# tugitbartlomiej/ViTParticleFilterTracker

Hardware: AMD Instinct MI355X
Metric: frames/sec @ 4096 particles, ViT-B/16 224px; 1/2/4/8 MI355X scaling (higher is better)
Workload: dtype bf16; 1 GPU; 4096 particles, vit_base_patch16_224 bf16, 224x224 frames, full tracking step per frame; particles=4096, particles_per_gpu=4096, arch=vit_base_patch16_224, hip_graph=True, parallelism=particle-shard x1

## Files before the change

vitparticlefiltertracker_amd/csrc/gemm_bf16.hip:

```cpp
#include <algorithm>
#include <atomic>
#include "gemm_common.h"

using namespace vpf;
using namespace vpf::gemm;

namespace {

constexpr int BK = 64;
constexpr int OPERAND_BYTES = BM * BK * 2;
static_assert(OPERAND_BYTES == TILE_BYTES, "bf16 K-tile geometry");
constexpr int AUX_PARTS = 15;
constexpr int MAX_PARTS = 16;
constexpr int AUX_BYTES = 2048 + AUX_PARTS * 2048;

template <int EPI, bool WIDE = false, bool OUT8 = false, bool PART = false>
__global__ __launch_bounds__(NTHREADS) void k_gemm_bf16(const bf16_t* __restrict__ A, int lda,
                                                        const bf16_t* __restrict__ W,
                                                        const float* __restrict__ bias,
                                                        const bf16_t* residual,
                                                        const float* __restrict__ pos, int g2,
                                                        const float2* __restrict__ stats,
                                                        const float* __restrict__ colsum,
                                                        bf16_t* C, int ldc, int M, int N, int K, int group,
// ... 131 lines not shown
    const int region = (wid >> 1) + ((wid >> 1) >= (nk % 3) ? 1 : 0);
    finish_tile<EPI, OUT8, DIRECT>(smem + region * OPERAND_BYTES + (wid & 1) * 16384, aux, acc, wm, wn, m0, n0, lane,
                                   residual, pos, g2, C, ldc, M, N, stats_out, stats_rows, o8);
}

template <int EPI, bool OUT8 = false>
__global__ __launch_bounds__(NTHREADS) void k_gemm_pp(const bf16_t* __restrict__ A, int lda,
                                                      const bf16_t* __restrict__ W,
                                                      const float* __restrict__ bias,
                                                      const bf16_t* residual,
                                                      const float* __restrict__ pos, int g2,
                                                      const float2* __restrict__ stats,
                                                      const float* __restrict__ colsum,
                                                      bf16_t* C, int ldc, int M, int N, int K, int group,
                                                      int stats_parts, float ln_eps, float* stats_out,
                                                      int stats_rows, Out8 o8) {
    constexpr int HALF = 16384;
    constexpr int RING = 8 * HALF;
    static_assert(RING + AUX_BYTES <= 160 * 1024, "LDS budget");
    __shared__ __attribute__((aligned(16))) char smem[RING + AUX_BYTES];
    const int tid = threadIdx.x, lane = tid & 63;
    const int wid = __builtin_amdgcn_readfirstlane(tid >> 6);
    const int wm = wid >> 2, wn = wid & 3;

    int m0, n0;
    tile_of(M, N, group, m0, n0);
    constexpr bool DIRECT = (EPI == VPF_EPI_LN_GELU || EPI == VPF_EPI_BIAS_GELU) && !OUT8;

    const char* Ablk = reinterpret_cast<const char*>(A) + (size_t)m0 * lda * 2;
    const char* Bblk = reinterpret_cast<const char*>(W) + (size_t)n0 * K * 2;
    uint32_t off[4][2];
#pragma unroll
    for (int p = 0; p < 2; ++p) {
        const int rho = (wid + 8 * p) * 8 + (lane >> 3);
        const int lch = (lane & 7) ^ ((rho >> 1) & 7);
        const int ra0 = (rho >> 6) * 128 + (rho & 63);
        const int rb0 = (rho >> 5) * 64 + (DIRECT ? wperm(rho & 31) : (rho & 31));
        const int ra[2] = {ra0, ra0 + 64}, rb[2] = {rb0, rb0 + 32};
#pragma unroll
        for (int h = 0; h < 2; ++h) {
            off[h == 0 ? 0 : 3][p] = (uint32_t)min(ra[h], M - 1 - m0) * (uint32_t)(lda * 2) + (uint32_t)(lch * 16);
            off[h == 0 ? 1 : 2][p] = (uint32_t)min(rb[h], N - 1 - n0) * (uint32_t)(K * 2) + (uint32_t)(lch * 16);
        }
    }
    const int nk = K / BK;
    auto stage = [&](int type, int kt) {
        kt = min(kt, nk - 1);
        char* slot = smem + ((kt & 1) * 4 + type) * HALF;
        const char* src = (type == 0 || type == 3) ? Ablk : Bblk;
        const uint32_t koff = (uint32_t)kt * (BK * 2);
#pragma unroll
        for (int p = 0; p < 2; ++p)
            __builtin_amdgcn_global_load_lds((gptr_t)(src + off[type][p] + koff), (lptr_t)(slot + (wid + 8 * p) * 1024),
                                             16, 0, 0);
    };

    constexpr bool LN = (EPI == VPF_EPI_LN || EPI == VPF_EPI_LN_GELU);
    char* aux = smem + RING;
    dma_bias_colsum<LN>(aux, bias, colsum, n0, N, wid, lane);
    if constexpr (LN) dma_planes(aux + 2048, stats, stats_parts, m0, M, wid, lane);
    stage(0, 0); stage(1, 0); stage(2, 0); stage(3, 0); stage(0, 1); stage(1, 1);
    asm volatile("s_waitcnt vmcnt(8)" ::: "memory");
    __builtin_amdgcn_s_barrier();
    if (wm == 1) __builtin_amdgcn_s_barrier();
    asm volatile("" ::: "memory");

    f32x4 acc[4][8];
#pragma unroll
    for (int j = 0; j < 4; ++j)
#pragma unroll
        for (int i = 0; i < 8; ++i) acc[j][i] = f32x4{0.f, 0.f, 0.f, 0.f};

    const int fr = lane & 15, fq = lane >> 4;
    const int sw = (fr >> 1) & 7;
    const int abase = (wm * 64 + fr) * 128, bbase = (wn * 32 + fr) * 128;
    auto mfma_quadrant = [&](const i32x4 (&fa)[2][4], const i32x4 (&fb)[2][2], int mh, int nh) {
        asm volatile("s_waitcnt lgkmcnt(0)" ::: "memory");
        __builtin_amdgcn_sched_barrier(0);
#pragma unroll
        for (int ks = 0; ks < 2; ++ks)
#pragma unroll
            for (int j = 0; j < 2; ++j)
#pragma unroll
                for (int i = 0; i < 4; ++i)
                    acc[nh * 2 + j][mh * 4 + i] = __builtin_amdgcn_mfma_f32_16x16x32_bf16(
                        __builtin_bit_cast(bf16x8, fb[ks][j]), __builtin_bit_cast(bf16x8, fa[ks][i]),
                        acc[nh * 2 + j][mh * 4 + i], 0, 0, 0);
        __builtin_amdgcn_sched_barrier(0);
    };
    auto read_a = [&](i32x4 (&fa)[2][4], const char* slot) {
#pragma unroll
        for (int ks = 0; ks < 2; ++ks)
#pragma unroll
            for (int i = 0; i < 4; ++i) fa[ks][i] = lds16(slot + abase + i * 2048 + (((ks * 4 + fq) ^ sw) << 4));
    };
    auto read_b = [&](i32x4 (&fb)[2][2], const char* slot) {
#pragma unroll
        for (int ks = 0; ks < 2; ++ks)
#pragma unroll
            for (int j = 0; j < 2; ++j) fb[ks][j] = lds16(slot + bbase + j * 2048 + (((ks * 4 + fq) ^ sw) << 4));
    };
    auto bar = [&]() {
        __builtin_amdgcn_sched_barrier(0);
        __builtin_amdgcn_s_barrier();
        __builtin_amdgcn_sched_barrier(0);
    };

    for (int kt = 0; kt < nk; ++kt) {
        const char* buf = smem + (kt & 1) * 4 * HALF;
        i32x4 fa0[2][4], fa1[2][4], fb0[2][2], fb1[2][2];
        read_a(fa0, buf);
        read_b(fb0, buf + HALF);
        stage(2, kt + 1);
        asm volatile("s_waitcnt vmcnt(8)" ::: "memory");
        bar();
        mfma_quadrant(fa0, fb0, 0, 0);
        bar();
        read_b(fb1, buf + 2 * HALF);
        stage(3, kt + 1);
        asm volatile("s_waitcnt vmcnt(8)" ::: "memory");
        bar();
        mfma_quadrant(fa0, fb1, 0, 1);
        bar();
        read_a(fa1, buf + 3 * HALF);
        stage(0, kt + 2);
        bar();
        mfma_quadrant(fa1, fb1, 1, 1);
        bar();
        stage(1, kt + 2);
        asm volatile("s_waitcnt vmcnt(8)" ::: "memory");
        bar();
        mfma_quadrant(fa1, fb0, 1, 0);
        bar();
    }
    if (wm == 0) __builtin_amdgcn_s_barrier();
    asm volatile("s_waitcnt vmcnt(0)" ::: "memory");

    if constexpr (LN) combine_planes(aux + 2048, aux, stats_parts, K, ln_eps, tid);
    finish_tile<EPI, OUT8, DIRECT>(smem + wid * 16384, aux, acc, wm, wn, m0, n0, lane, residual, pos, g2, C, ldc, M, N,
                                   stats_out, stats_rows, o8);
}

constexpr int WALK_HALF = 16384;
constexpr int WALK_RING = 8 * WALK_HALF;
constexpr int WALK_GROUP_IMG = 2048;
constexpr int walk_aux_set(int epi) { return epi == VPF_EPI_BIAS_RESIDUAL ? 1024 : 4096; }
constexpr int walk_smem(int epi) {
    return WALK_RING + 2 * walk_aux_set(epi) + (epi_is_gelu(epi) ? 0 : 8 * WALK_GROUP_IMG);
}
constexpr bool walk_reads_early(int epi) {
    return epi == VPF_EPI_LN || epi == VPF_EPI_LN_GELU || epi == VPF_EPI_BIAS_RESIDUAL;
}

template <int OFF>
__device__ __forceinline__ i32x4 lds16_at(uint32_t addr) {
    static_assert(OFF >= 0 && OFF < 65536, "ds_read offset field");
    i32x4 v;
    asm volatile("ds_read_b128 %0, %1 offset:%2" : "=v"(v) : "v"(addr), "n"(OFF));
    return v;
}
template <int SLOT, int NF>
__device__ __forceinline__ void frag_read(i32x4 (&f)[2][NF], const uint32_t (&ad)[2]) {
#pragma unroll
    for (int ks = 0; ks < 2; ++ks) {
        f[ks][0] = lds16_at<SLOT>(ad[ks]);
        f[ks][1] = lds16_at<SLOT + 2048>(ad[ks]);
        if constexpr (NF == 4) {
            f[ks][2] = lds16_at<SLOT + 4096>(ad[ks]);
            f[ks][3] = lds16_at<SLOT + 6144>(ad[ks]);
        }
    }
}

template <int EPI, bool EARLY = walk_reads_early(EPI)>
__device__ __forceinline__ void gemm_walk_body(char* smem, const bf16_t* __restrict__ A, int lda,
                                               const bf16_t* __restrict__ W, const float* __restrict__ bias,
                                               const float2* __restrict__ stats, const float* __restrict__ colsum,
                                               const bf16_t* residual, bf16_t* C, int ldc, int M, int N, int K,
                                               int group, int tiles, float* stats_out) {
    constexpr bool RES = EPI == VPF_EPI_BIAS_RESIDUAL;
    constexpr bool DIRECT = epi_is_gelu(EPI);
    constexpr int HALF = WALK_HALF;
    constexpr int RING = WALK_RING;
    constexpr int AUX_SET = walk_aux_set(EPI);
    constexpr int GROUP_IMG = WALK_GROUP_IMG;
    const int tid = threadIdx.x, lane = tid & 63;
    const int wid = __builtin_amdgcn_readfirstlane(tid >> 6);
    const int wm = wid >> 2, wn = wid & 3;
    constexpr bool LN = epi_is_ln(EPI);
    const int nk = K / BK;

    const int stride = (int)gridDim.x >> 3;
    int lid = xcd_first(tiles, (int)blockIdx.x & 7) + ((int)blockIdx.x >> 3);
    const int lid_end = xcd_first(tiles, ((int)blockIdx.x & 7) + 1);
    if (lid >= lid_end) return;
    int m0, n0;
    tile_of_lid(M, N, group, lid, m0, n0);

    const char* Ablk;
    const char* Bblk;
    uint32_t off[4][2];
    auto set_panels = [&](int tm0, int tn0, int ln) {
        Ablk = reinterpret_cast<const char*>(A) + (size_t)tm0 * lda * 2;
        Bblk = reinterpret_cast<const char*>(W) + (size_t)tn0 * K * 2;
#pragma unroll
        for (int p = 0; p < 2; ++p) {
            const int rho = (wid + 8 * p) * 8 + (ln >> 3);
            const int lch = (ln & 7) ^ ((rho >> 1) & 7);
            const int ra0 = (rho >> 6) * 128 + (rho & 63);
            const int rb0 = (rho >> 5) * 64 + (DIRECT ? wperm(rho & 31) : (rho & 31));
            const int ra[2] = {ra0, ra0 + 64}, rb[2] = {rb0, rb0 + 32};
#pragma unroll
            for (int h = 0; h < 2; ++h) {
                off[h == 0 ? 0 : 3][p] = (uint32_t)min(ra[h], M - 1 - tm0) * (uint32_t)(lda * 2) + (uint32_t)(lch * 16);
                off[h == 0 ? 1 : 2][p] = (uint32_t)min(rb[h], N - 1 - tn0) * (uint32_t)(K * 2) + (uint32_t)(lch * 16);
            }
        }
    };
    auto stage = [&](int type, int kt) {
        kt = min(kt, nk - 1);
        char* slot = smem + ((kt & 1) * 4 + type) * HALF;
        const char* src = (type == 0 || type == 3) ? Ablk : Bblk;
        const uint32_t koff = (uint32_t)kt * (BK * 2);
#pragma unroll
        for (int p = 0; p < 2; ++p)
            __builtin_amdgcn_global_load_lds((gptr_t)(src + off[type][p] + koff), (lptr_t)(slot + (wid + 8 * p) * 1024),
                                             16, 0, 0);
    };
    auto load_aux = [&](char* dst, int tm0, int tn0, int ln) {
        dma_bias_colsum<LN>(dst, bias, colsum, tn0, N, wid, ln);
        if constexpr (LN) dma_planes(dst + 2048, stats, 0, tm0, M, wid, ln);
    };

    set_panels(m0, n0, lane);
    load_aux(smem + RING, m0, n0, lane);
    stage(0, 0); stage(1, 0); stage(2, 0); stage(3, 0); stage(0, 1); stage(1, 1);
    asm volatile("s_waitcnt vmcnt(8)" ::: "memory");
    __builtin_amdgcn_s_barrier();
    asm volatile("" ::: "memory");

    f32x4 acc[4][8];
    const int fr = lane & 15, fq = lane >> 4;
    const int sw = (fr >> 1) & 7;
    const int abase = (wm * 64 + fr) * 128, bbase = (wn * 32 + fr) * 128;
    auto mfma_quadrant = [&](const i32x4 (&fa)[2][4], const i32x4 (&fb)[2][2], int mh, int nh) {
        asm volatile("s_waitcnt lgkmcnt(0)" ::: "memory");
        __builtin_amdgcn_sched_barrier(0);
#pragma unroll
        for (int ks = 0; ks < 2; ++ks)
#pragma unroll
            for (int j = 0; j < 2; ++j)
#pragma unroll
                for (int i = 0; i < 4; ++i)
                    acc[nh * 2 + j][mh * 4 + i] = __builtin_amdgcn_mfma_f32_16x16x32_bf16(
                        __builtin_bit_cast(bf16x8, fb[ks][j]), __builtin_bit_cast(bf16x8, fa[ks][i]),
                        acc[nh * 2 + j][mh * 4 + i], 0, 0, 0);
        __builtin_amdgcn_sched_barrier(0);
    };
    auto read_a = [&](i32x4 (&fa)[2][4], const char* slot) {
#pragma unroll
        for (int ks = 0; ks < 2; ++ks)
#pragma unroll
            for (int i = 0; i < 4; ++i) fa[ks][i] = lds16(slot + abase + i * 2048 + (((ks * 4 + fq) ^ sw) << 4));
    };
    auto read_b = [&](i32x4 (&fb)[2][2], const char* slot) {
#pragma unroll
        for (int ks = 0; ks < 2; ++ks)
#pragma unroll
            for (int j = 0; j < 2; ++j) fb[ks][j] = lds16(slot + bbase + j * 2048 + (((ks * 4 + fq) ^ sw) << 4));
    };
    auto bar = [&]() {
        __builtin_amdgcn_sched_barrier(0);
        __builtin_amdgcn_s_barrier();
        __builtin_amdgcn_sched_barrier(0);
    };
    i32x4 fa0[2][4];
    const uint32_t ring32 = (uint32_t)(uintptr_t)(lptr_t)smem;
    const uint32_t arel[2] = {(uint32_t)(abase + ((fq ^ sw) << 4)), (uint32_t)(abase + (((4 + fq) ^ sw) << 4))};
    const uint32_t brel[2] = {(uint32_t)(bbase + ((fq ^ sw) << 4)), (uint32_t)(bbase + (((4 + fq) ^ sw) << 4))};

    int skt = 0;
    int par = 0;
    for (;;) {
        const int lid_next = lid + stride;
        const bool more = lid_next < lid_end;
        int m0n = m0, n0n = n0;
        if constexpr (EARLY) {
            const uint32_t a0[2] = {ring32 + arel[0], ring32 + arel[1]};
            frag_read<0>(fa0, a0);
            __builtin_amdgcn_sched_barrier(0);
        }
        if (wm == 1) __builtin_amdgcn_s_barrier();
        asm volatile("" ::: "memory");
#pragma unroll
        for (int j = 0; j < 4; ++j)
#pragma unroll
            for (int i = 0; i < 8; ++i) acc[j][i] = f32x4{0.f, 0.f, 0.f, 0.f};

        for (int kt = 0; kt < nk; ++kt, ++skt) {
            const char* buf = smem + (kt & 1) * 4 * HALF;
            i32x4 fa1[2][4], fb0[2][2], fb1[2][2];
            const uint32_t buf32 = ring32 + (kt & 1) * 4 * HALF, nbuf32 = ring32 + ((kt + 1) & 1) * 4 * HALF;
            [[maybe_unused]] const uint32_t ad[2] = {buf32 + arel[0], buf32 + arel[1]};
            [[maybe_unused]] const uint32_t bd[2] = {buf32 + brel[0], buf32 + brel[1]};
            [[maybe_unused]] const uint32_t nad[2] = {nbuf32 + arel[0], nbuf32 + arel[1]};
            if constexpr (EARLY) {
                frag_read<HALF>(fb0, bd);
            } else {
                read_a(fa0, buf);
                read_b(fb0, buf + HALF);
            }
            stage(2, skt + 1);
            asm volatile("s_waitcnt vmcnt(8)" ::: "memory");
            bar();
            mfma_quadrant(fa0, fb0, 0, 0);
            bar();
            if constexpr (EARLY) frag_read<2 * HALF>(fb1, bd);
            else read_b(fb1, buf + 2 * HALF);
            stage(3, skt + 1);
            asm volatile("s_waitcnt vmcnt(8)" ::: "memory");
            bar();
            mfma_quadrant(fa0, fb1, 0, 1);
            bar();
            if (more && kt == nk - 2) {
                const int ln = opaque_lane();
                tile_of_lid(M, N, group, lid_next, m0n, n0n);
                set_panels(m0n, n0n, ln);
                load_aux(smem + RING + (par ^ 1) * AUX_SET, m0n, n0n, ln);
                skt -= nk;
            }
            if constexpr (EARLY) frag_read<3 * HALF>(fa1, ad);
            else read_a(fa1, buf + 3 * HALF);
            stage(0, skt + 2);
            if constexpr (EARLY) asm volatile("s_waitcnt vmcnt(8)" ::: "memory");
            bar();
            mfma_quadrant(fa1, fb1, 1, 1);
            bar();
            if constexpr (EARLY) frag_read<0>(fa0, nad);
            stage(1, skt + 2);
            asm volatile("s_waitcnt vmcnt(8)" ::: "memory");
            bar();
            mfma_quadrant(fa1, fb0, 1, 0);
            bar();
        }
        [[maybe_unused]] uint4 res[16];
        [[maybe_unused]] int eln = lane;
        if constexpr (RES) {
            eln = opaque_lane();
            load_residual<true>(res, residual, wm, wn, m0, n0, eln, ldc, M, N);
        } else if constexpr (EARLY && !DIRECT) {
            eln = opaque_lane();
        }
        if (wm == 0) __builtin_amdgcn_s_barrier();
        asm volatile("" ::: "memory");
        if constexpr (DIRECT)
            store_wave_tile_direct<EPI, true>(smem + RING + par * AUX_SET, acc, wm, wn, m0, n0, lane, C, ldc, M, N);
        else if constexpr (RES)
            store_wave_tile_group_res(smem + RING + 2 * AUX_SET + wid * GROUP_IMG, smem + RING + par * AUX_SET, acc, wm,
                                      wn, m0, n0, eln, res, C, ldc, M, N, stats_out, M);
        else
            store_wave_tile_group<EPI>(smem + RING + 2 * AUX_SET + wid * GROUP_IMG, smem + RING + par * AUX_SET, acc, wm,
                                       wn, m0, n0, eln, C, ldc, M, N);
        if (!more) break;
        lid = lid_next;
        m0 = m0n;
        n0 = n0n;
        par ^= 1;
    }
    asm volatile("s_waitcnt vmcnt(0)" ::: "memory");
}

template <int EPI>
__global__ __launch_bounds__(NTHREADS) void k_gemm_walk(const bf16_t* __restrict__ A, int lda,
                                                        const bf16_t* __restrict__ W,
                                                        const float* __restrict__ bias,
                                                        const float2* __restrict__ stats,
                                                        const float* __restrict__ colsum, bf16_t* C, int ldc, int M,
                                                        int N, int K, int group, int tiles) {
    static_assert(EPI == VPF_EPI_LN_GELU || EPI == VPF_EPI_BIAS_GELU || EPI == VPF_EPI_LN, "FC1's and QKV's epilogues");
    __shared__ __attribute__((aligned(16))) char smem[walk_smem(EPI)];
    gemm_walk_body<EPI>(smem, A, lda, W, bias, stats, colsum, nullptr, C, ldc, M, N, K, group, tiles, nullptr);
}

__global__ __launch_bounds__(NTHREADS) void k_gemm_walk_res(const bf16_t* __restrict__ A, int lda,
                                                            const bf16_t* __restrict__ W,
                                                            const float* __restrict__ bias, const bf16_t* residual,
                                                            bf16_t* C, int ldc, int M, int N, int K, int group,
                                                            int tiles, float* stats_out) {
    __shared__ __attribute__((aligned(16))) char smem[walk_smem(VPF_EPI_BIAS_RESIDUAL)];
    gemm_walk_body<VPF_EPI_BIAS_RESIDUAL>(smem, A, lda, W, bias, nullptr, nullptr, residual, C, ldc, M, N, K, group,
                                          tiles, stats_out);
}

}

#define VPF_IS_LN(E) ((E) == VPF_EPI_LN || (E) == VPF_EPI_LN_GELU)
#define VPF_IS_PROD(E) ((E) == VPF_EPI_BIAS_RESIDUAL || (E) == VPF_EPI_PATCH)
#define VPF_GEMM_ARGS                                                                                        \
    A, (int)lda, W, bias, residual, pos, patch_rows, reinterpret_cast<const float2*>(row_stats), colsum, C,     \
        (int)ldc, m, n, k, group, stats_parts, ln_eps, stats_out, stats_rows, o8
#define VPF_GEMM_LAUNCH(E)                                                                                   \
    do {                                                                                                     \
        if (kern == 5 && !(VPF_IS_LN(E) && stats_parts > AUX_PARTS) && o8.q == nullptr)                      \
            hipLaunchKernelGGL((k_gemm_pp<E, false>), grid, block, 0, s, VPF_GEMM_ARGS);                     \
        else if (kern == 5 && VPF_IS_PROD(E) && o8.q != nullptr)                                             \
            hipLaunchKernelGGL((k_gemm_pp<E, VPF_IS_PROD(E)>), grid, block, 0, s, VPF_GEMM_ARGS);            \
        else if (VPF_IS_LN(E) && stats_parts > AUX_PARTS)                                                    \
            hipLaunchKernelGGL((k_gemm_bf16<E, VPF_IS_LN(E)>), grid, block, 0, s, VPF_GEMM_ARGS);             \
        else if (VPF_IS_PROD(E) && o8.q != nullptr)                                                          \
            hipLaunchKernelGGL((k_gemm_bf16<E, false, VPF_IS_PROD(E)>), grid, block, 0, s, VPF_GEMM_ARGS);    \
        else                                                                                                 \
            hipLaunchKernelGGL((k_gemm_bf16<E>), grid, block, 0, s, VPF_GEMM_ARGS);                           \
    } while (0)

constexpr int kDefaultGroup = 4;
static int g_kernel = 0;
static int g_group = -1;
static int gemm_kernel_for(int epilogue) {
    if (g_kernel) return g_kernel;
    return (epilogue == VPF_EPI_LN || epilogue == VPF_EPI_LN_GELU) ? 5 : 1;
}
static int tile_group_for(int64_t N, int epilogue) {
    if (g_group >= 0) return g_group;
    if (N <= 1024) return 2;
    return epilogue == VPF_EPI_LN_GELU ? 8 : kDefaultGroup;
}
int vpf_gemm_tile_group() { return g_group >= 0 ? g_group : kDefaultGroup; }
int vpf_gemm_tile_group_mx8(int epilogue) {
    if (g_group >= 0) return g_group;
    return epilogue == VPF_EPI_LN ? 8 : kDefaultGroup;
}
VPF_API int vpf_gemm_tune(int kernel, int group) {
    if (kernel != 0 && kernel != 1 && kernel != 5) return VPF_ERR_ARG;
    if (group < -1 || group > 64) return VPF_ERR_ARG;
    g_kernel = kernel;
    g_group = kernel == 0 ? -1 : group;
    return 0;
}

static bool walk_by_default(int epilogue, int64_t nk) {
    if (epilogue == VPF_EPI_BIAS_RESIDUAL) return nk == 12 || nk == 48;
    return epilogue == VPF_EPI_LN_GELU || epilogue == VPF_EPI_LN;
}
static int g_walk_mode = 0;
static int g_walk_cap = 0;
static std::atomic<int> g_walk_cus[64];
static int walk_device_grid() {
    int dev = 0;
    if (hipGetDevice(&dev) != hipSuccess || dev < 0 || dev >= 64) return 0;
    int cus = g_walk_cus[dev].load(std::memory_order_relaxed);
    if (cus == 0) {
        if (hipDeviceGetAttribute(&cus, hipDeviceAttributeMultiprocessorCount, dev) != hipSuccess) return 0;
        cus &= ~7;
        g_walk_cus[dev].store(cus, std::memory_order_relaxed);
    }
    return cus;
}
static int walk_grid_for(int epilogue, int64_t tiles, int64_t K, int stats_parts) {
    if (epilogue != VPF_EPI_LN_GELU && epilogue != VPF_EPI_BIAS_GELU && epilogue != VPF_EPI_LN &&
        epilogue != VPF_EPI_BIAS_RESIDUAL)
        return 0;
    if (g_kernel != 0 || g_walk_mode < 0 || (g_walk_mode == 0 && !walk_by_default(epilogue, K / BK))) return 0;
    if ((K / BK) % 2 != 0 || stats_parts != 0 || tiles < 8) return 0;
    int grid = walk_device_grid();
    if (g_walk_cap > 0) grid = std::min(grid, g_walk_cap);
    if (grid < 8) return 0;
    if (g_walk_mode == 0) return tiles >= 2 * (int64_t)grid ? grid : 0;
    return (int)std::min<int64_t>(grid, tiles & ~(int64_t)7);
}
VPF_API int vpf_gemm_persistent(int mode, int grid_cap) {
    if (mode < -1 || mode > 1 || grid_cap < 0 || grid_cap % 8 != 0 || grid_cap > 4096) return VPF_ERR_ARG;
    g_walk_mode = mode;
    g_walk_cap = grid_cap;
    (void)walk_device_grid();
    return 0;
}
VPF_API int vpf_gemm_persistent_grid(int64_t M, int64_t N, int64_t K, int epilogue, int stats_parts) {
    (void)walk_device_grid();
    if (M <= 0 || N <= 0 || K <= 0 || K % BK != 0) return 0;
    const int64_t tiles = ((M + BM - 1) / BM) * ((N + BN - 1) / BN);
    return tiles > INT32_MAX ? 0 : walk_grid_for(epilogue, tiles, K, stats_parts);
}

int vpf_check_out8(const uint8_t* C8, int64_t ld8, const uint32_t* Cs, int64_t lds_c, int64_t rows, int64_t N) {
    if (!C8) return Cs ? VPF_ERR_ARG : 0;
    if (!Cs || N % 128 != 0 || ld8 < N || ld8 % 8 != 0 || ((uintptr_t)C8 & 7) || lds_c < rows || lds_c % 64 != 0 ||
        ((uintptr_t)Cs & 3) || ld8 > INT32_MAX || lds_c > INT32_MAX / 4)
        return VPF_ERR_ARG;
    return 0;
}

int64_t vpf_gemm_check(int64_t M, int64_t N, int64_t K, int64_t k_unit, int64_t lda, int a_align, int a_bytes,
                       bool has_c, int64_t ldc, const float* bias, const float* colsum, const float* row_stats) {
    if (M <= 0 || N <= 0 || K <= 0 || K % k_unit != 0 || N % 8 != 0 || lda < K || lda % a_align != 0) return 0;
    if (has_c && (ldc < N || ldc % 8 != 0 || ldc > INT32_MAX / 2)) return 0;
    if (M > INT32_MAX / 2 || N > 65536 || K > 65536 || lda > INT32_MAX / 2) return 0;
    if ((uint64_t)BM * (uint64_t)lda * (uint64_t)a_bytes > UINT32_MAX) return 0;
    if (((uintptr_t)bias & 15) || ((uintptr_t)colsum & 15) || ((uintptr_t)row_stats & 7)) return 0;
    const int64_t tiles = ((M + BM - 1) / BM) * ((N + BN - 1) / BN);
    return tiles > INT32_MAX ? 0 : tiles;
}

VPF_API int vpf_gemm_bf16(const uint16_t* A, int64_t lda, const uint16_t* W, const float* bias,
                          const uint16_t* residual, const float* pos, int patch_rows, const float* row_stats,
                          const float* colsum, uint16_t* C, int64_t ldc, int64_t M, int64_t N, int64_t K,
                          int epilogue, int stats_parts, float ln_eps, float* stats_out, uint8_t* C8, int64_t ld8,
                          uint32_t* Cs, int64_t lds_c, void* stream) {
    const int64_t tiles = vpf_gemm_check(M, N, K, BK, lda, 8, 2, true, ldc, bias, colsum, row_stats);
    if (!tiles) return VPF_ERR_ARG;
    if (!A || !W || !bias || !C) return VPF_ERR_ARG;
    if (epilogue == VPF_EPI_BIAS_RESIDUAL && !residual) return VPF_ERR_ARG;
    if (epilogue == VPF_EPI_PATCH && (!pos || patch_rows <= 0 || M % patch_rows != 0)) return VPF_ERR_ARG;
    if ((epilogue == VPF_EPI_LN || epilogue == VPF_EPI_LN_GELU) && (!row_stats || !colsum)) return VPF_ERR_ARG;
// ... 159 lines not shown
```

vitparticlefiltertracker_amd/csrc/gemm_common.h:

```cpp
#pragma once
#include "vpf_common.h"
#include "mx8.h"
#include "../../include/vpf.h"

int vpf_gemm_tile_group();
int vpf_gemm_tile_group_mx8(int epilogue);
int vpf_check_out8(const uint8_t* C8, int64_t ld8, const uint32_t* Cs, int64_t lds_c, int64_t rows, int64_t N);
int64_t vpf_gemm_check(int64_t M, int64_t N, int64_t K, int64_t k_unit, int64_t lda, int a_align, int a_bytes,
                       bool has_c, int64_t ldc, const float* bias, const float* colsum, const float* row_stats);

namespace vpf {
namespace gemm {

typedef const __attribute__((address_space(1))) void* gptr_t;
typedef __attribute__((address_space(3))) void* lptr_t;
typedef short bf16x8 __attribute__((ext_vector_type(8)));
typedef int i32x4 __attribute__((ext_vector_type(4)));

__device__ __forceinline__ i32x4 lds16(const char* p) {
    i32x4 v;
    asm volatile("ds_read_b128 %0, %1" : "=v"(v) : "v"((uint32_t)(uintptr_t)(lptr_t)p));
    return v;
}
typedef int i32x2 __attribute__((ext_vector_type(2)));
__device__ __forceinline__ i32x2 lds8(const void* p) {
    i32x2 v;
    asm volatile("ds_read_b64 %0, %1" : "=v"(v) : "v"((uint32_t)(uintptr_t)(lptr_t)p));
    return v;
}
__device__ __forceinline__ int lds4(const void* p) {
    int v;
    asm volatile("ds_read_b32 %0, %1" : "=v"(v) : "v"((uint32_t)(uintptr_t)(lptr_t)p));
    return v;
}
__device__ __forceinline__ int opaque_lane() {
    int l;
    asm volatile("v_mbcnt_lo_u32_b32 %0, -1, 0\n\tv_mbcnt_hi_u32_b32 %0, -1, %0" : "=v"(l));
    return l;
}
typedef float f32x4 __attribute__((ext_vector_type(4)));
typedef float f32x2 __attribute__((ext_vector_type(2)));

constexpr int BM = 256, BN = 256;
constexpr int NTHREADS = 512;
constexpr int TILE_BYTES = BM * 128;

typedef unsigned u32x4_nt __attribute__((ext_vector_type(4)));
__device__ __forceinline__ void st16_nt(void* p, uint4 v) {
    __builtin_nontemporal_store(u32x4_nt{v.x, v.y, v.z, v.w}, reinterpret_cast<u32x4_nt*>(p));
}

__device__ __forceinline__ void tile_of_lid(int M, int N, int group, int lid, int& m0, int& n0) {
    const int tiles_n = (N + BN - 1) / BN;
    int tm, tn;
    if (group > 0) {
        const int tiles_m = (M + BM - 1) / BM;
        const int per_group = group * tiles_n;
        const int g = lid / per_group, idx = lid - g * per_group;
        const int gm0 = g * group;
        const int gsz = min(group, tiles_m - gm0);
        tn = idx / gsz;
        tm = gm0 + (idx - tn * gsz);
    } else {
        tm = lid / tiles_n;
        tn = lid - tm * tiles_n;
    }
    m0 = tm * BM;
    n0 = tn * BN;
}
__device__ __forceinline__ int xcd_first(int nwg, int xcd) {
    const int q = nwg >> 3, r = nwg & 7;
    return xcd < r ? xcd * (q + 1) : r * (q + 1) + (xcd - r) * q;
}
__device__ __forceinline__ void tile_of(int M, int N, int group, int& m0, int& n0) {
    const int nwg = gridDim.x, bid = blockIdx.x;
    tile_of_lid(M, N, group, xcd_first(nwg, bid & 7) + (bid >> 3), m0, n0);
}

__device__ __forceinline__ f32x2 gelu_sig2(f32x2 x) {
    constexpr float L2E = 1.4426950408889634f;
    constexpr float c1 = -1.6003141571059616f * L2E, c2 = -0.06940178687219423f * L2E;
    const f32x2 q = (x * x) * c2 + c1;
    const f32x2 t = x * q;
    const f32x2 d = f32x2{__builtin_amdgcn_exp2f(t.x), __builtin_amdgcn_exp2f(t.y)} + 1.0f;
    return x * f32x2{__builtin_amdgcn_rcpf(d.x), __builtin_amdgcn_rcpf(d.y)};
}

struct Out8 {
    uint8_t* q;
    uint8_t* s;
    int ldq, lds;
};

constexpr bool epi_is_ln(int epi) { return epi == VPF_EPI_LN || epi == VPF_EPI_LN_GELU; }
constexpr bool epi_is_gelu(int epi) { return epi == VPF_EPI_BIAS_GELU || epi == VPF_EPI_LN_GELU; }

template <bool LN>
__device__ __forceinline__ void dma_bias_colsum(char* aux, const float* __restrict__ bias,
                                                const float* __restrict__ colsum, int n0, int N, int wid, int lane) {
    if (wid == 0)
        __builtin_amdgcn_global_load_lds((gptr_t)(bias + min(n0 + lane * 4, N - 4)), (lptr_t)aux, 16, 0, 0);
    if constexpr (LN) {
        if (wid == 1)
            __builtin_amdgcn_global_load_lds((gptr_t)(colsum + min(n0 + lane * 4, N - 4)), (lptr_t)(aux + 1024), 16, 0, 0);
    }
}
__device__ __forceinline__ void dma_planes(char* dst, const float2* __restrict__ stats, int stats_parts, int m0, int M,
                                           int wid, int lane) {
    const float* sd = reinterpret_cast<const float*>(stats);
    const int planes = stats_parts > 0 ? stats_parts : 1;
    if ((M & 1) == 0 && ((uintptr_t)sd & 15) == 0) {
        for (int pc = wid; pc < 2 * planes; pc += 8) {
            const int p = pc >> 1, hf = pc & 1;
            __builtin_amdgcn_global_load_lds(
                (gptr_t)(sd + (int64_t)p * 2 * M + min(2 * m0 + hf * 256 + lane * 4, 2 * M - 4)),
                (lptr_t)(dst + p * 2048 + hf * 1024), 16, 0, 0);
        }
    } else {
        for (int p = 0; p < planes; ++p)
            __builtin_amdgcn_global_load_lds(
                (gptr_t)(sd + (int64_t)p * 2 * M + min(2 * m0 + wid * 64 + lane, 2 * M - 1)),
                (lptr_t)(dst + p * 2048 + wid * 256), 4, 0, 0);
    }
}
__device__ __forceinline__ void combine_planes(const char* planes_lds, char* aux, int stats_parts, int K, float ln_eps,
                                               int tid) {
    if (stats_parts > 0 && tid < BM) {
        float sm = 0.f, sq = 0.f;
        for (int p = 0; p < stats_parts; ++p) {
            const float2 st = *reinterpret_cast<const float2*>(planes_lds + p * 2048 + tid * 8);
            sm += st.x;
            sq += st.y;
        }
        const float inv_k = 1.0f / (float)K;
        const float mean = sm * inv_k;
        const float var = fmaxf(fmaf(sq, inv_k, -mean * mean), 0.f);
        *reinterpret_cast<float2*>(aux + 2048 + tid * 8) = make_float2(mean, __builtin_amdgcn_rsqf(var + ln_eps));
    }
}

struct EpiCols { float4 b, c; };
struct EpiRow { f32x2 rstd, nrm; };
struct Frag4 { f32x2 lo, hi; };
template <bool LN>
__device__ __forceinline__ EpiCols epi_cols(const char* aux, int col) {
    EpiCols v;
    v.b = *reinterpret_cast<const float4*>(aux + col * 4);
    v.c = LN ? *reinterpret_cast<const float4*>(aux + 1024 + col * 4) : make_float4(0.f, 0.f, 0.f, 0.f);
    return v;
}
template <bool LN>
__device__ __forceinline__ EpiRow epi_row(const char* aux, int row) {
    if constexpr (LN) {
        const float2 st = *reinterpret_cast<const float2*>(aux + 2048 + row * 8);
        return EpiRow{f32x2{st.y, st.y}, f32x2{-st.y * st.x, -st.y * st.x}};
    } else {
        return EpiRow{f32x2{1.f, 1.f}, f32x2{0.f, 0.f}};
    }
}
template <int EPI>
__device__ __forceinline__ Frag4 epi_math4(const f32x4& a, const EpiCols& cl, const EpiRow& rw) {
    f32x2 v01, v23;
    const f32x2 a01 = {a[0], a[1]}, a23 = {a[2], a[3]};
    const f32x2 b01 = {cl.b.x, cl.b.y}, b23 = {cl.b.z, cl.b.w};
    if constexpr (epi_is_ln(EPI)) {
        const f32x2 c01 = {cl.c.x, cl.c.y}, c23 = {cl.c.z, cl.c.w};
        v01 = __builtin_elementwise_fma(rw.rstd, a01, __builtin_elementwise_fma(rw.nrm, c01, b01));
        v23 = __builtin_elementwise_fma(rw.rstd, a23, __builtin_elementwise_fma(rw.nrm, c23, b23));
    } else {
        v01 = a01 + b01;
        v23 = a23 + b23;
    }
    if constexpr (epi_is_gelu(EPI)) {
        v01 = gelu_sig2(v01);
// ... 101 lines not shown
    }
}

template <int EPI>
__device__ __forceinline__ void store_wave_tile_pipe(char* img, const char* aux, const f32x4 (&acc)[4][8], int wm,
                                                     int wn, int m0, int n0, int lane, const uint4 (&res)[16],
                                                     bf16_t* C, int ldc, int M, int N, float* stats_out,
                                                     int stats_rows) {
    constexpr bool LN = epi_is_ln(EPI);
    constexpr bool RES = EPI == VPF_EPI_BIAS_RESIDUAL;
    const int fr = lane & 15, fq = lane >> 4, c16 = lane & 7;
    bf16_t* Cl = C + (int64_t)(m0 + wm * 128 + 2 * (lane >> 3)) * ldc + (n0 + wn * 64 + c16 * 8);
    EpiCols cl[4];
#pragma unroll
    for (int j = 0; j < 4; ++j) cl[j] = epi_cols<LN>(aux, wn * 64 + j * 16 + fq * 4);
#pragma unroll
    for (int i = 0; i < 8; ++i) {
        const EpiRow rw = epi_row<LN>(aux, wm * 128 + i * 16 + fr);
#pragma unroll
        for (int j = 0; j < 4; ++j) epi_to_image4<EPI>(img, i * 16 + fr, j * 4 + fq, acc[j][i], cl[j], rw);
        __builtin_amdgcn_wave_barrier();
#pragma unroll
        for (int h = 0; h < 2; ++h) {
            const int row = i * 16 + 2 * (lane >> 3) + h;
            uint4 v = image_get16(img, row, c16, h == 1);
            const int m = m0 + wm * 128 + row;
            const int n = n0 + wn * 64 + c16 * 8;
            const bool ok = m < M && n < N;
            if constexpr (RES) {
                const uint4 rv = res[2 * i + h];
                const uint32_t w[4] = {v.x, v.y, v.z, v.w};
                const uint32_t rr[4] = {rv.x, rv.y, rv.z, rv.w};
                uint32_t o[4];
#pragma unroll
                for (int e = 0; e < 4; ++e)
                    o[e] = pack_bf2(bf2f((bf16_t)(w[e] & 0xffff)) + bf2f((bf16_t)(rr[e] & 0xffff)),
                                    bf2f((bf16_t)(w[e] >> 16)) + bf2f((bf16_t)(rr[e] >> 16)));
                v = make_uint4(o[0], o[1], o[2], o[3]);
                if (stats_out != nullptr) park_row_partial(img, row, c16, v, ok);
            }
            if (ok) {
                if constexpr (RES) *reinterpret_cast<uint4*>(Cl + (int64_t)(i * 16 + h) * ldc) = v;
                else st16_nt(Cl + (int64_t)(i * 16 + h) * ldc, v);
            }
        }
    }
    if constexpr (RES) {
        const int nb = n0 + wn * 64;
        if (stats_out != nullptr && nb < N) {
            __builtin_amdgcn_wave_barrier();
            float4 t = make_float4(0.f, 0.f, 0.f, 0.f);
#pragma unroll
            for (int q = 0; q < 4; ++q) {
                const float4 u0 = *reinterpret_cast<const float4*>(img + (2 * lane) * 128 + q * 16);
                const float4 u1 = *reinterpret_cast<const float4*>(img + (2 * lane + 1) * 128 + q * 16);
                t.x += u0.x + u0.z; t.y += u0.y + u0.w;
                t.z += u1.x + u1.z; t.w += u1.y + u1.w;
            }
            float* plane = stats_out + (int64_t)(nb >> 6) * stats_rows * 2;
            const int m = m0 + wm * 128 + 2 * lane;
            if (m + 1 < M) *reinterpret_cast<float4*>(plane + (int64_t)m * 2) = t;
            else if (m < M) *reinterpret_cast<float2*>(plane + (int64_t)m * 2) = make_float2(t.x, t.y);
        }
    }
}

__device__ __forceinline__ void lds_write8(const void* p, uint2 v) {
    const i32x2 w = {(int)v.x, (int)v.y};
    asm volatile("ds_write_b64 %0, %1" ::"v"((uint32_t)(uintptr_t)(lptr_t)p), "v"(w) : "memory");
}
template <int EPI>
__device__ __forceinline__ void store_wave_tile_group(char* img, const char* aux, const f32x4 (&acc)[4][8], int wm,
                                                      int wn, int m0, int n0, int lane, bf16_t* C, int ldc, int M,
                                                      int N) {
    static_assert(EPI == VPF_EPI_LN, "group image: the LN fold without GELU (QKV)");
    const int fr = lane & 15, fq = lane >> 4, c16 = lane & 7, r8 = lane >> 3;
    bf16_t* Cl = C + (int64_t)(m0 + wm * 128 + 2 * r8) * ldc + (n0 + wn * 64 + c16 * 8);
    i32x4 cb[4], cc[4];
    i32x2 st[8];
#pragma unroll
    for (int j = 0; j < 4; ++j) {
        const int col = wn * 64 + j * 16 + fq * 4;
        cb[j] = lds16(aux + col * 4);
        cc[j] = lds16(aux + 1024 + col * 4);
    }
#pragma unroll
    for (int i = 0; i < 8; ++i) st[i] = lds8(aux + 2048 + (wm * 128 + i * 16 + fr) * 8);
    asm volatile("s_waitcnt lgkmcnt(0)" : "+v"(cb[0]), "+v"(cb[1]), "+v"(cb[2]), "+v"(cb[3])::"memory");
    asm volatile("" : "+v"(cc[0]), "+v"(cc[1]), "+v"(cc[2]), "+v"(cc[3])::"memory");
    asm volatile("" : "+v"(st[0]), "+v"(st[1]), "+v"(st[2]), "+v"(st[3]), "+v"(st[4]), "+v"(st[5]), "+v"(st[6]),
                   "+v"(st[7])::"memory");
    EpiCols cl[4];
#pragma unroll
    for (int j = 0; j < 4; ++j) cl[j] = EpiCols{__builtin_bit_cast(float4, cb[j]), __builtin_bit_cast(float4, cc[j])};
    const char* wr = img + fr * 128;
    const char* rd = img + (2 * r8) * 128 + ((c16 ^ r8) << 4);
    const int n = n0 + wn * 64 + c16 * 8;
    i32x4 pend[2];
    auto store_group = [&](int i) {
        asm volatile("" : "+v"(pend[0]), "+v"(pend[1])::"memory");
#pragma unroll
        for (int h = 0; h < 2; ++h) {
            uint4 v = __builtin_bit_cast(uint4, pend[h]);
            if (h == 1) { const uint32_t t0 = v.x, t1 = v.y; v.x = v.z; v.y = v.w; v.z = t0; v.w = t1; }
            const int m = m0 + wm * 128 + i * 16 + 2 * r8 + h;
            if (m < M && n < N) st16_nt(Cl + (int64_t)(i * 16 + h) * ldc, v);
        }
    };
#pragma unroll
    for (int i = 0; i < 8; ++i) {
        const float2 s2 = __builtin_bit_cast(float2, st[i]);
        const EpiRow rw = EpiRow{f32x2{s2.y, s2.y}, f32x2{-s2.y * s2.x, -s2.y * s2.x}};
        uint2 pk[4];
#pragma unroll
        for (int j = 0; j < 4; ++j) pk[j] = epi_pack4<EPI>(acc[j][i], cl[j], rw);
#pragma unroll
        for (int j = 0; j < 4; ++j) lds_write8(wr + (((j * 4 + fq) ^ fr) << 3), pk[j]);
        asm volatile("s_waitcnt lgkmcnt(0)" ::: "memory");
        if (i > 0) store_group(i - 1);
        pend[0] = lds16(rd);
        pend[1] = lds16(rd + 128);
    }
    asm volatile("s_waitcnt lgkmcnt(0)" ::: "memory");
    store_group(7);
}

__device__ __forceinline__ float2 row_partial8(uint4 v, bool ok) {
    typedef __bf16 bf16x2_t __attribute__((ext_vector_type(2)));
    const uint32_t w[4] = {v.x, v.y, v.z, v.w};
    const bf16x2_t one2 = __builtin_bit_cast(bf16x2_t, 0x3F803F80u);
    float s1 = 0.f, s2 = 0.f;
#pragma unroll
    for (int e = 0; e < 4; ++e) {
        const bf16x2_t pr = __builtin_bit_cast(bf16x2_t, w[e]);
        s1 = __builtin_amdgcn_fdot2_f32_bf16(pr, one2, s1, false);
        s2 = __builtin_amdgcn_fdot2_f32_bf16(pr, pr, s2, false);
    }
    if (!ok) { s1 = 0.f; s2 = 0.f; }
    return make_float2(s1, s2);
}
template <int SHL>
__device__ __forceinline__ float dpp_row_shl(float x) {
    return __builtin_bit_cast(float, __builtin_amdgcn_update_dpp(0, __builtin_bit_cast(int, x), 0x100 + SHL, 0xF, 0xF, true));
}
__device__ __forceinline__ float row8_sum(float p) {
    const float q = p + dpp_row_shl<1>(p);
    float t = 0.f;
    t += q;
    t += dpp_row_shl<2>(q);
    t += dpp_row_shl<4>(q);
    t += dpp_row_shl<6>(q);
    return t;
}
__device__ __forceinline__ void store_wave_tile_group_res(char* img, const char* aux, const f32x4 (&acc)[4][8], int wm,
                                                          int wn, int m0, int n0, int lane, const uint4 (&res)[16],
                                                          bf16_t* C, int ldc, int M, int N, float* stats_out,
                                                          int stats_rows) {
    constexpr int EPI = VPF_EPI_BIAS_RESIDUAL;
    const int fr = lane & 15, fq = lane >> 4, c16 = lane & 7, r8 = lane >> 3;
    bf16_t* Cl = C + (int64_t)(m0 + wm * 128 + 2 * r8) * ldc + (n0 + wn * 64 + c16 * 8);
    i32x4 cb[4];
#pragma unroll
    for (int j = 0; j < 4; ++j) cb[j] = lds16(aux + (wn * 64 + j * 16 + fq * 4) * 4);
    asm volatile("s_waitcnt lgkmcnt(0)" : "+v"(cb[0]), "+v"(cb[1]), "+v"(cb[2]), "+v"(cb[3])::"memory");
    EpiCols cl[4];
#pragma unroll
    for (int j = 0; j < 4; ++j) cl[j] = EpiCols{__builtin_bit_cast(float4, cb[j]), make_float4(0.f, 0.f, 0.f, 0.f)};
    const EpiRow rw = EpiRow{f32x2{1.f, 1.f}, f32x2{0.f, 0.f}};
    const char* wr = img + fr * 128;
    const char* rd = img + (2 * r8) * 128 + ((c16 ^ r8) << 4);
    const int n = n0 + wn * 64 + c16 * 8;
    const int nb = n0 + wn * 64;
    const bool planes = stats_out != nullptr && nb < N;
    float* pl = stats_out + ((int64_t)(nb >> 6) * stats_rows + (m0 + wm * 128 + 2 * r8)) * 2;
    i32x4 pend[2];
    auto store_group = [&](int i) {
        asm volatile("" : "+v"(pend[0]), "+v"(pend[1])::"memory");
        const int m = m0 + wm * 128 + i * 16 + 2 * r8;
        uint4 v[2];
#pragma unroll
        for (int h = 0; h < 2; ++h) {
            v[h] = __builtin_bit_cast(uint4, pend[h]);
            if (h == 1) { const uint32_t t0 = v[h].x, t1 = v[h].y; v[h].x = v[h].z; v[h].y = v[h].w; v[h].z = t0; v[h].w = t1; }
            v[h] = add_bf16x8(v[h], res[2 * i + h]);
            if (m + h < M && n < N) *reinterpret_cast<uint4*>(Cl + (int64_t)(i * 16 + h) * ldc) = v[h];
        }
        if (planes) {
            const float2 p0 = row_partial8(v[0], m < M && n < N), p1 = row_partial8(v[1], m + 1 < M && n < N);
            const float4 t = make_float4(row8_sum(p0.x), row8_sum(p0.y), row8_sum(p1.x), row8_sum(p1.y));
            if (c16 == 0) {
                if (m + 1 < M) *reinterpret_cast<float4*>(pl + i * 32) = t;
                else if (m < M) *reinterpret_cast<float2*>(pl + i * 32) = make_float2(t.x, t.y);
            }
        }
    };
#pragma unroll
    for (int i = 0; i < 8; ++i) {
        uint2 pk[4];
#pragma unroll
        for (int j = 0; j < 4; ++j) pk[j] = epi_pack4<EPI>(acc[j][i], cl[j], rw);
#pragma unroll
        for (int j = 0; j < 4; ++j) lds_write8(wr + (((j * 4 + fq) ^ fr) << 3), pk[j]);
        asm volatile("s_waitcnt lgkmcnt(0)" ::: "memory");
        if (i > 0) store_group(i - 1);
        pend[0] = lds16(rd);
        pend[1] = lds16(rd + 128);
    }
    asm volatile("s_waitcnt lgkmcnt(0)" ::: "memory");
    store_group(7);
}

__device__ __forceinline__ int wperm(int r) {
    return (r & ~31) | (((r >> 2) & 3) << 3) | (((r >> 4) & 1) << 2) | (r & 3);
}

template <int EPI, bool DMA_LIVE = false>
__device__ __forceinline__ void store_wave_tile_direct(const char* aux, const f32x4 (&acc)[4][8], int wm, int wn, int m0,
                                                       int n0, int lane, bf16_t* C, int ldc, int M, int N) {
    static_assert(epi_is_gelu(EPI), "direct stores: the GELU epilogues");
    constexpr bool LN = epi_is_ln(EPI);
    const int fr = lane & 15, fq = lane >> 4;
    bf16_t* Cl = C + (int64_t)(m0 + wm * 128 + fr) * ldc + (n0 + wn * 64 + fq * 8);
    EpiCols cl[4];
    EpiRow rws[8];
    if constexpr (DMA_LIVE) {
        i32x4 cb[4], cc[4];
        i32x2 st[8];
#pragma unroll
        for (int j = 0; j < 4; ++j) {
            const int col = wn * 64 + (j >> 1) * 32 + fq * 8 + (j & 1) * 4;
            cb[j] = lds16(aux + col * 4);
            if constexpr (LN) cc[j] = lds16(aux + 1024 + col * 4);
        }
        if constexpr (LN) {
#pragma unroll
            for (int i = 0; i < 8; ++i) st[i] = lds8(aux + 2048 + (wm * 128 + i * 16 + fr) * 8);
        }
        asm volatile("s_waitcnt lgkmcnt(0)" : "+v"(cb[0]), "+v"(cb[1]), "+v"(cb[2]), "+v"(cb[3])::"memory");
        if constexpr (LN) {
            asm volatile("" : "+v"(cc[0]), "+v"(cc[1]), "+v"(cc[2]), "+v"(cc[3])::"memory");
            asm volatile("" : "+v"(st[0]), "+v"(st[1]), "+v"(st[2]), "+v"(st[3]), "+v"(st[4]), "+v"(st[5]), "+v"(st[6]),
                           "+v"(st[7])::"memory");
        }
#pragma unroll
        for (int j = 0; j < 4; ++j) {
            cl[j].b = __builtin_bit_cast(float4, cb[j]);
            cl[j].c = LN ? __builtin_bit_cast(float4, cc[j]) : make_float4(0.f, 0.f, 0.f, 0.f);
        }
#pragma unroll
        for (int i = 0; i < 8; ++i) {
            if constexpr (LN) {
                const float2 s2 = __builtin_bit_cast(float2, st[i]);
                rws[i] = EpiRow{f32x2{s2.y, s2.y}, f32x2{-s2.y * s2.x, -s2.y * s2.x}};
            } else {
                rws[i] = EpiRow{f32x2{1.f, 1.f}, f32x2{0.f, 0.f}};
            }
        }
    } else {
#pragma unroll
        for (int j = 0; j < 4; ++j) cl[j] = epi_cols<LN>(aux, wn * 64 + (j >> 1) * 32 + fq * 8 + (j & 1) * 4);
    }
#pragma unroll
    for (int i = 0; i < 8; ++i) {
        EpiRow rw;
        if constexpr (DMA_LIVE) rw = rws[i];
        else rw = epi_row<LN>(aux, wm * 128 + i * 16 + fr);
        const int m = m0 + wm * 128 + i * 16 + fr;
#pragma unroll
        for (int h = 0; h < 2; ++h) {
            const uint2 lo = epi_pack4<EPI>(acc[2 * h][i], cl[2 * h], rw);
            const uint2 hi = epi_pack4<EPI>(acc[2 * h + 1][i], cl[2 * h + 1], rw);
            const int n = n0 + wn * 64 + h * 32 + fq * 8;
            if (m < M && n < N)
                *reinterpret_cast<uint4*>(Cl + (int64_t)(i * 16) * ldc + h * 32) = make_uint4(lo.x, lo.y, hi.x, hi.y);
        }
    }
}

template <bool PAR = true>
__device__ __forceinline__ void load_residual(uint4 (&res)[16], const bf16_t* residual, int wm, int wn, int m0,
                                              int n0, int lane, int ldc, int M, int N) {
    const int c16 = lane & 7;
    const int n = n0 + wn * 64 + c16 * 8;
    const bf16_t* rl = residual + (int64_t)(m0 + wm * 128 + (PAR ? 2 : 1) * (lane >> 3)) * ldc + n;
#pragma unroll
    for (int it = 0; it < 16; ++it) {
        const int roff = PAR ? (it >> 1) * 16 + (it & 1) : it * 8;
        const int m = m0 + wm * 128 + roff + (PAR ? 2 : 1) * (lane >> 3);
        res[it] = (m < M && n < N) ? *reinterpret_cast<const uint4*>(rl + (int64_t)roff * ldc) : make_uint4(0, 0, 0, 0);
    }
}

template <int EPI, bool OUT8>
__device__ __forceinline__ void store_wave_tile(char* img, const char* aux, const f32x4 (&acc)[4][8], int wm, int wn,
                                                int m0, int n0, int lane, const uint4 (&res)[16],
                                                const float* __restrict__ pos, int g2, bf16_t* C, int ldc, int M,
                                                int N, float* stats_out, int stats_rows, Out8 o8) {
    epi_to_image<EPI>(img, aux, acc, wm, wn, lane);
    const int c16 = lane & 7;
    constexpr bool PROD = (EPI == VPF_EPI_BIAS_RESIDUAL || EPI == VPF_EPI_PATCH);
    constexpr bool GATHER8 = OUT8 && EPI != VPF_EPI_PATCH;
    uint32_t e8s[16];
    __builtin_amdgcn_wave_barrier();
#pragma unroll
    for (int it = 0; it < 16; ++it) {
        const int row = it * 8 + (lane >> 3);
        uint4 v = image_get16(img, row, c16, row & 1);
        const int m = m0 + wm * 128 + row;
        const int n = n0 + wn * 64 + c16 * 8;
        const bool ok = m < M && n < N;
        int64_t orow = m;
        if constexpr (EPI == VPF_EPI_PATCH) {
            const int pi = m % g2;
            orow = (int64_t)(m / g2) * (g2 + 1) + 1 + pi;
            const float* pr = pos + (int64_t)(1 + pi) * N + min(n, N - 8);
            const float4 p0 = *reinterpret_cast<const float4*>(pr);
            const float4 p1 = *reinterpret_cast<const float4*>(pr + 4);
            const uint32_t w[4] = {v.x, v.y, v.z, v.w};
            const float pv[8] = {p0.x, p0.y, p0.z, p0.w, p1.x, p1.y, p1.z, p1.w};
            uint32_t o[4];
#pragma unroll
            for (int e = 0; e < 4; ++e)
                o[e] = pack_bf2(bf2f((bf16_t)(w[e] & 0xffff)) + pv[2 * e], bf2f((bf16_t)(w[e] >> 16)) + pv[2 * e + 1]);
            v = make_uint4(o[0], o[1], o[2], o[3]);
        }
        if constexpr (EPI == VPF_EPI_BIAS_RESIDUAL) v = add_bf16x8(v, res[it]);
        if constexpr (PROD) {
            if (stats_out != nullptr) park_row_partial(img, row, c16, v, ok);
        }
        if constexpr (OUT8) {
            uint32_t e8;
            const uint2 q = mx8_quant8(v, e8);
            e8s[it] = e8;
            if (ok) {
                *reinterpret_cast<uint2*>(o8.q + orow * o8.ldq + n) = q;
                if (!GATHER8 && (c16 & 3) == 0) o8.s[mx8_scale_byte(orow, n, o8.lds)] = (uint8_t)e8;
            }
        }
        if (ok && C != nullptr) *reinterpret_cast<uint4*>(C + orow * ldc + n) = v;
    }
    if constexpr (GATHER8) {
        __builtin_amdgcn_wave_barrier();
        if ((c16 & 3) == 0) {
#pragma unroll
            for (int it = 0; it < 16; ++it) {
                const int row = it * 8 + (lane >> 3);
                const int w = (row >> 6) * 32 + (c16 >> 2) * 16 + (row & 15);
                img[(w >> 4) * 128 + 64 + (w & 15) * 4 + ((row >> 4) & 3)] = (char)e8s[it];
            }
        }
        __builtin_amdgcn_wave_barrier();
        const uint32_t word = *reinterpret_cast<const uint32_t*>(img + (lane >> 4) * 128 + 64 + (lane & 15) * 4);
        store_scale_word(o8, word, m0 + wm * 128, n0 + wn * 64, M, N, lane >> 5, (lane >> 4) & 1, lane & 15);
    }
    if constexpr (PROD)
        store_row_stats<EPI == VPF_EPI_PATCH>(img, stats_out, stats_rows, m0 + wm * 128, n0 + wn * 64, lane, M, N, g2);
}

__device__ __forceinline__ int wperm16(int r) {
    return (r & ~63) | (((r >> 2) & 3) << 4) | (((r >> 4) & 3) << 2) | (r & 3);
}

// ... 98 lines not shown
```

Measured before the change: 8.000 frames/s.

## Stream residual tiles through LDS FIFO in bias-residual GEMM epilogue

Replaces the up-front register load of all 16 residual vectors per wave with a two-slot LDS FIFO filled by global_load_lds. Residual rows for later groups are issued while earlier groups are packed and stored, and counted vmcnt waits keep the loads in flight. It also adds full-tile template specialisations that drop per-row bounds checks and the stats-plane branch. The intent is to cut register pressure and epilogue latency, at the cost of extra LDS traffic, more complex wait accounting and reuse of ring LDS space that could be racy.

```diff
diff --git a/vitparticlefiltertracker_amd/csrc/gemm_bf16.hip b/vitparticlefiltertracker_amd/csrc/gemm_bf16.hip
--- a/vitparticlefiltertracker_amd/csrc/gemm_bf16.hip
+++ b/vitparticlefiltertracker_amd/csrc/gemm_bf16.hip
@@ -307,13 +307,6 @@
     return epi == VPF_EPI_LN || epi == VPF_EPI_LN_GELU || epi == VPF_EPI_BIAS_RESIDUAL;
 }
 
-template <int OFF>
-__device__ __forceinline__ i32x4 lds16_at(uint32_t addr) {
-    static_assert(OFF >= 0 && OFF < 65536, "ds_read offset field");
-    i32x4 v;
-    asm volatile("ds_read_b128 %0, %1 offset:%2" : "=v"(v) : "v"(addr), "n"(OFF));
-    return v;
-}
 template <int SLOT, int NF>
 __device__ __forceinline__ void frag_read(i32x4 (&f)[2][NF], const uint32_t (&ad)[2]) {
 #pragma unroll
@@ -498,11 +491,20 @@
             mfma_quadrant(fa1, fb0, 1, 0);
             bar();
         }
-        [[maybe_unused]] uint4 res[16];
+        [[maybe_unused]] ResFifo rf;
+        [[maybe_unused]] bool full_wave_tile = false;
         [[maybe_unused]] int eln = lane;
         if constexpr (RES) {
             eln = opaque_lane();
-            load_residual<true>(res, residual, wm, wn, m0, n0, eln, ldc, M, N);
+            const int mb = min(m0 + wm * 128, M - 1), nb = min(n0 + wn * 64, N - 8);
+            full_wave_tile = m0 + wm * 128 + 128 <= M && n0 + wn * 64 + 64 <= N;
+            rf.ldc2 = (int64_t)ldc * 2;
+            rf.r2 = 2 * (eln >> 3);
+            rf.rmax = M - 1 - mb;
+            rf.src = reinterpret_cast<const char*>(residual + (int64_t)mb * ldc + nb) + min((eln & 7) * 16, (N - 8 - nb) * 2);
+            rf.lds = smem + (4 + 2) * HALF + wid * 1024;
+            rf.issue<true, HALF>(0);
+            rf.issue<true, HALF>(1);
         } else if constexpr (EARLY && !DIRECT) {
             eln = opaque_lane();
         }
@@ -510,10 +512,19 @@
         asm volatile("" ::: "memory");
         if constexpr (DIRECT)
             store_wave_tile_direct<EPI, true>(smem + RING + par * AUX_SET, acc, wm, wn, m0, n0, lane, C, ldc, M, N);
-        else if constexpr (RES)
-            store_wave_tile_group_res(smem + RING + 2 * AUX_SET + wid * GROUP_IMG, smem + RING + par * AUX_SET, acc, wm,
-                                      wn, m0, n0, eln, res, C, ldc, M, N, stats_out, M);
-        else
+        else if constexpr (RES) {
+            char* img = smem + RING + 2 * AUX_SET + wid * GROUP_IMG;
+            const char* aux = smem + RING + par * AUX_SET;
+            if (full_wave_tile && stats_out != nullptr)
+                store_wave_tile_group_res<true, true, HALF>(img, aux, acc, wm, wn, m0, n0, eln, rf, C, ldc, M, N,
+                                                            stats_out, M);
+            else if (full_wave_tile)
+                store_wave_tile_group_res<true, false, HALF>(img, aux, acc, wm, wn, m0, n0, eln, rf, C, ldc, M, N,
+                                                             stats_out, M);
+            else
+                store_wave_tile_group_res<false, false, HALF>(img, aux, acc, wm, wn, m0, n0, eln, rf, C, ldc, M, N,
+                                                              stats_out, M);
+        } else
             store_wave_tile_group<EPI>(smem + RING + 2 * AUX_SET + wid * GROUP_IMG, smem + RING + par * AUX_SET, acc, wm,
                                        wn, m0, n0, eln, C, ldc, M, N);
         if (!more) break;
diff --git a/vitparticlefiltertracker_amd/csrc/gemm_common.h b/vitparticlefiltertracker_amd/csrc/gemm_common.h
--- a/vitparticlefiltertracker_amd/csrc/gemm_common.h
+++ b/vitparticlefiltertracker_amd/csrc/gemm_common.h
@@ -20,6 +20,13 @@
 __device__ __forceinline__ i32x4 lds16(const char* p) {
     i32x4 v;
     asm volatile("ds_read_b128 %0, %1" : "=v"(v) : "v"((uint32_t)(uintptr_t)(lptr_t)p));
+    return v;
+}
+template <int OFF>
+__device__ __forceinline__ i32x4 lds16_at(uint32_t addr) {
+    static_assert(OFF >= 0 && OFF < 65536, "ds_read offset field");
+    i32x4 v;
+    asm volatile("ds_read_b128 %0, %1 offset:%2" : "=v"(v) : "v"(addr), "n"(OFF));
     return v;
 }
 typedef int i32x2 __attribute__((ext_vector_type(2)));
@@ -427,11 +434,35 @@
     t += dpp_row_shl<6>(q);
     return t;
 }
+template <int N_>
+__device__ __forceinline__ void wait_vmcnt() {
+    asm volatile("s_waitcnt vmcnt(%0)" ::"n"(N_) : "memory");
+}
+template <int I>
+struct IntC { static constexpr int value = I; };
+constexpr int RES_DEFER = 2;
+struct ResFifo {
+    const char* src;
+    int64_t ldc2;
+    int r2, rmax;
+    char* lds;
+    template <bool CLAMP, int HALF_STRIDE>
+    __device__ __forceinline__ void issue(int i) const {
+#pragma unroll
+        for (int h = 0; h < 2; ++h) {
+            const int row = i * 16 + r2 + h;
+            __builtin_amdgcn_global_load_lds((gptr_t)(src + (int64_t)(CLAMP ? min(row, rmax) : row) * ldc2),
+                                             (lptr_t)(lds + (i & 1) * HALF_STRIDE + h * 8192), 16, 0, 0);
+        }
+    }
+};
+template <bool FULL, bool PLANES, int HALF_STRIDE>
 __device__ __forceinline__ void store_wave_tile_group_res(char* img, const char* aux, const f32x4 (&acc)[4][8], int wm,
-                                                          int wn, int m0, int n0, int lane, const uint4 (&res)[16],
+                                                          int wn, int m0, int n0, int lane, const ResFifo& rf,
                                                           bf16_t* C, int ldc, int M, int N, float* stats_out,
                                                           int stats_rows) {
     constexpr int EPI = VPF_EPI_BIAS_RESIDUAL;
+    constexpr int S = 2 + (PLANES ? 1 : 0);
     const int fr = lane & 15, fq = lane >> 4, c16 = lane & 7, r8 = lane >> 3;
     bf16_t* Cl = C + (int64_t)(m0 + wm * 128 + 2 * r8) * ldc + (n0 + wn * 64 + c16 * 8);
     i32x4 cb[4];
@@ -446,43 +477,59 @@
     const char* rd = img + (2 * r8) * 128 + ((c16 ^ r8) << 4);
     const int n = n0 + wn * 64 + c16 * 8;
     const int nb = n0 + wn * 64;
-    const bool planes = stats_out != nullptr && nb < N;
+    const bool planes = FULL ? PLANES : (stats_out != nullptr && nb < N);
     float* pl = stats_out + ((int64_t)(nb >> 6) * stats_rows + (m0 + wm * 128 + 2 * r8)) * 2;
-    i32x4 pend[2];
-    auto store_group = [&](int i) {
-        asm volatile("" : "+v"(pend[0]), "+v"(pend[1])::"memory");
-        const int m = m0 + wm * 128 + i * 16 + 2 * r8;
+    const uint32_t fifo_rd = (uint32_t)(uintptr_t)(lptr_t)rf.lds + (uint32_t)lane * 16;
+    i32x4 pend[RES_DEFER][2], rr[2];
+    auto finish_group = [&](auto gc) {
+        constexpr int g = decltype(gc)::value;
+        wait_vmcnt<!FULL ? 0 : g == 0 ? 2 : g == 1 ? 2 + S : g == 7 ? 2 * S : 2 + 2 * S>();
+        rr[0] = lds16_at<(g & 1) * HALF_STRIDE>(fifo_rd);
+        rr[1] = lds16_at<(g & 1) * HALF_STRIDE + 8192>(fifo_rd);
+        asm volatile("s_waitcnt lgkmcnt(0)" : "+v"(rr[0]), "+v"(rr[1])::"memory");
+        if constexpr (g + 2 < 8) {
+            rf.template issue<!FULL, HALF_STRIDE>(g + 2);
+            asm volatile("" ::: "memory");
+            __builtin_amdgcn_sched_barrier(0);
+        }
+        i32x4(&pd)[2] = pend[g % RES_DEFER];
+        asm volatile("" : "+v"(pd[0]), "+v"(pd[1])::"memory");
+        const int m = m0 + wm * 128 + g * 16 + 2 * r8;
         uint4 v[2];
 #pragma unroll
         for (int h = 0; h < 2; ++h) {
-            v[h] = __builtin_bit_cast(uint4, pend[h]);
+            v[h] = __builtin_bit_cast(uint4, pd[h]);
             if (h == 1) { const uint32_t t0 = v[h].x, t1 = v[h].y; v[h].x = v[h].z; v[h].y = v[h].w; v[h].z = t0; v[h].w = t1; }
-            v[h] = add_bf16x8(v[h], res[2 * i + h]);
-            if (m + h < M && n < N) *reinterpret_cast<uint4*>(Cl + (int64_t)(i * 16 + h) * ldc) = v[h];
+            v[h] = add_bf16x8(v[h], __builtin_bit_cast(uint4, rr[h]));
+            if (FULL || (m + h < M && n < N)) *reinterpret_cast<uint4*>(Cl + (int64_t)(g * 16 + h) * ldc) = v[h];
         }
         if (planes) {
-            const float2 p0 = row_partial8(v[0], m < M && n < N), p1 = row_partial8(v[1], m + 1 < M && n < N);
+            const float2 p0 = row_partial8(v[0], FULL || (m < M && n < N)),
+                         p1 = row_partial8(v[1], FULL || (m + 1 < M && n < N));
             const float4 t = make_float4(row8_sum(p0.x), row8_sum(p0.y), row8_sum(p1.x), row8_sum(p1.y));
             if (c16 == 0) {
-                if (m + 1 < M) *reinterpret_cast<float4*>(pl + i * 32) = t;
-                else if (m < M) *reinterpret_cast<float2*>(pl + i * 32) = make_float2(t.x, t.y);
+                if (FULL || m + 1 < M) *reinterpret_cast<float4*>(pl + g * 32) = t;
+                else if (m < M) *reinterpret_cast<float2*>(pl + g * 32) = make_float2(t.x, t.y);
             }
         }
     };
-#pragma unroll
-    for (int i = 0; i < 8; ++i) {
+    auto step = [&](auto ic) {
+        constexpr int i = decltype(ic)::value;
         uint2 pk[4];
 #pragma unroll
         for (int j = 0; j < 4; ++j) pk[j] = epi_pack4<EPI>(acc[j][i], cl[j], rw);
 #pragma unroll
         for (int j = 0; j < 4; ++j) lds_write8(wr + (((j * 4 + fq) ^ fr) << 3), pk[j]);
-        asm volatile("s_waitcnt lgkmcnt(0)" ::: "memory");
-        if (i > 0) store_group(i - 1);
-        pend[0] = lds16(rd);
-        pend[1] = lds16(rd + 128);
-    }
-    asm volatile("s_waitcnt lgkmcnt(0)" ::: "memory");
-    store_group(7);
+        if constexpr (i >= RES_DEFER) finish_group(IntC<i - RES_DEFER>{});
+        else asm volatile("s_waitcnt lgkmcnt(0)" ::: "memory");
+        pend[i % RES_DEFER][0] = lds16(rd);
+        pend[i % RES_DEFER][1] = lds16(rd + 128);
+    };
+    step(IntC<0>{}); step(IntC<1>{}); step(IntC<2>{}); step(IntC<3>{});
+    step(IntC<4>{}); step(IntC<5>{}); step(IntC<6>{}); step(IntC<7>{});
+    if constexpr (RES_DEFER >= 3) finish_group(IntC<5>{});
+    if constexpr (RES_DEFER >= 2) finish_group(IntC<6>{});
+    finish_group(IntC<7>{});
 }
 
 __device__ __forceinline__ int wperm(int r) {
```

Result: no change. 8.042 frames/s (median of 6 runs) (+0.5%).
